# PANXIONG-CN/TEC-MoLLM

Hardware: AMD Instinct MI355X
Metric: train samples/sec (higher is better)
Workload: dtype f32; 1 GPU; BASELINE configs[1]: B=8/GPU, L_in=48, L_out=12, N=2911, F=10 (d_emb=12), 3 GPT-2 blocks, full fwd+bwd+AdamW, fp32, GATv2 per_timestep, dropout on (p=0.1); global_batch=8, parallelism=dp1, data_feed=fixed, launch=eager

## Files before the change

__graft_entry__.py:

```python
from __future__ import annotations

import concurrent.futures as cf
import os
import re
import subprocess
import sys

ROOT = os.path.dirname(os.path.abspath(__file__))
PKG = os.path.join(ROOT, "tec-mollm_amd")
CSRC = os.path.join(PKG, "csrc")
OUT_LIB = os.path.join(PKG, "tecmollm", "libtecmollm_hip.so")
OBJ_DIR = os.path.join(CSRC, "build")
SOURCES = ["gemm.hip", "gemm_mk_nk.hip", "gemm_mk_kn.hip", "gemm_km_kn.hip", "gemm_bf16_mk_nk.hip", "gemm_bf16_mk_kn.hip", "gemm_bf16_km_kn.hip", "gemm_bf16_dma.hip", "gemm_bf16_p8.hip", "gemm_bf16_tn.hip", "gemm_bf16_res_mk.hip", "gemm_bf16_res_km.hip", "gemm_x3.hip", "conv_seq.hip", "conv_dw_seq.hip", "norm.hip", "attention.hip", "attention_long.hip", "spatial_fwd.hip", "spatial_fwd2.hip", "spatial_bwd.hip", "spatial_bwd2.hip", "misc.hip", "trainstep.hip", "baselines.hip", "util.cpp"]
HIPCC = os.environ.get("HIPCC", "/opt/rocm/bin/hipcc")
FLAGS = ["--offload-arch=gfx950", "-O3", "-std=c++17", "-fPIC", "-Wno-pass-failed", "-Wno-unused-value"]


def _ensure_path():
    for p in (ROOT, PKG):
        if p not in sys.path:
            sys.path.insert(0, p)


def _stale(target: str, deps) -> bool:
    if not os.path.exists(target):
        return True
    t = os.path.getmtime(target)
    return any(os.path.getmtime(d) > t for d in deps)


def _compile(src: str) -> str:
    obj = os.path.join(OBJ_DIR, os.path.splitext(src)[0] + ".o")
    deps = [os.path.join(CSRC, src), os.path.join(CSRC, "common.h"), os.path.join(CSRC, "spatial_common.h"), os.path.join(CSRC, "spatial2_common.h"), os.path.join(CSRC, "gemm_impl.h"), os.path.join(CSRC, "gemm_bf16_impl.h"), os.path.join(CSRC, "gemm_x3_impl.h"), os.path.join(CSRC, "gemm_bf16_p8_loop.h"), os.path.join(CSRC, "attention_long.h"), os.path.join(ROOT, "include", "tecmollm.h")]
    if src in SPILL_CEILINGS:
        deps.append(os.path.abspath(__file__))
    if _stale(obj, deps):
        extra = ["-Rpass-analysis=kernel-resource-usage"] if src in SPILL_CEILINGS else []
        cmd = [HIPCC, *FLAGS, *extra, "-x", "hip", "-c", os.path.join(CSRC, src), "-o", obj]
        r = subprocess.run(cmd, capture_output=True, text=True)
        if r.returncode != 0:
            raise RuntimeError(f"hipcc failed on {src}:\n{r.stderr[-4000:]}")
        if src in SPILL_CEILINGS:
            try:
                check_spill_ceilings(src, r.stderr, SPILL_CEILINGS[src])
            except RuntimeError:
                os.remove(obj)
                raise
    return obj


SPILL_CEILINGS = {
    "conv_dw_seq.hip": [("conv_dw_seq_kernel", "ScratchSize [bytes/lane]", 0)],
    "attention.hip": [("attention_bwd_kernel_qstreamILi24ELb0ELb0E", "VGPRs Spill", 92),
                      ("attention_bwd_kernel_qstreamILi24ELb1ELb0E", "VGPRs Spill", 18),
                      ("attention_bwd_kernel_qstreamILi24ELb1ELb1E", "VGPRs Spill", 18)],
    "attention_long.hip": [("att_long_fwd_kernelILb0E", "ScratchSize [bytes/lane]", 0),
                           ("att_long_fwd_kernelILb1E", "ScratchSize [bytes/lane]", 0),
                           ("att_long_bwd_kernelILb0ELb0E", "ScratchSize [bytes/lane]", 0),
                           ("att_long_bwd_kernelILb1ELb0E", "ScratchSize [bytes/lane]", 0),
                           ("att_long_bwd_kernelILb1ELb1E", "ScratchSize [bytes/lane]", 0)],
}


def check_spill_ceilings(src: str, remarks: str, rules) -> None:
    name, bad, seen = None, [], {}
    for line in remarks.splitlines():
        if "Function Name:" in line:
            name = line.split("Function Name:")[1].split()[0]
            continue
        for frag, field, ceiling in rules:
            if name and frag in name and f"{field}:" in line:
                value = int(line.split(f"{field}:")[1].split()[0])
                seen[frag] = seen.get(frag, 0) + 1
                if value > ceiling:
                    bad.append(f"{name}: {field} {value} > {ceiling}")
    missing = [frag for frag, _, _ in rules if not seen.get(frag)]
    if bad or missing:
        raise RuntimeError(f"{src}: kernel resource ceilings exceeded {bad}; no remark for {missing}")


_VREG = re.compile(r"\bv(\d+)\b|\bv\[(\d+):(\d+)\]")


def _vregs(text: str) -> set:
    out = set()
# ... 117 lines not shown
```

include/tecmollm.h:

```cpp
#ifndef TECMOLLM_H
#define TECMOLLM_H

#include <stdint.h>

#ifdef __cplusplus
extern "C" {
#endif

#define TECM_OK 0
#define TECM_E_ARG (-1)
#define TECM_E_ALIGN (-2)
#define TECM_E_LAUNCH (-3)
#define TECM_E_LDS (-4)

#define TECM_ABI_VERSION 19
int tecm_abi_version(void);
const char* tecm_last_error(void);

typedef struct TecmWin {
  int32_t enabled;
  int32_t N;
  int32_t Lin, Lout;
  int32_t stride_t;
  int32_t taps;
  int32_t Cw;
  int32_t pad;
} TecmWin;

typedef struct TecmDrop {
  float p;
  int32_t _pad;
  uint64_t seed;
  int64_t ld;
  const uint64_t* seed_dev;
} TecmDrop;

enum { TECM_A_MK = 0, TECM_A_KM = 1 };
enum { TECM_B_NK = 0, TECM_B_KN = 1 };
enum { TECM_ACT_NONE = 0, TECM_ACT_GELU_ERF = 1, TECM_ACT_GELU_TANH = 2 };

#define TECM_IO_A_BF16 1
#define TECM_IO_B_BF16 2
#define TECM_IO_C_BF16 4
#define TECM_IO_PRE_BF16 8
typedef struct TecmGemm {
  int64_t M, N, K;
  const float* A; int64_t lda; int32_t a_layout; int32_t io_bf16; TecmWin a_win; TecmDrop a_drop;
  const float* B; int64_t ldb; int32_t b_layout; int32_t _p1; TecmWin b_win; TecmDrop b_drop;
// ... 128 lines not shown
int tecm_conv_weight_unpack(const float* dpack, float* dw, int32_t Cout, int32_t Cin, int32_t k,
                            void* stream);

typedef struct TecmConvDx {
  const void* dy;
  const void* wpack;
  float* dinp;
  int32_t B, Lc, N, Cout, ld_in, _pad;
} TecmConvDx;
int tecm_conv_dx_pack(const float* w3, const float* w5, const float* w7, void* wpack, int32_t Cout, int32_t Cin,
                      int32_t ld_in, void* stream);
int tecm_conv_dx_bf16(const TecmConvDx* p, void* stream);
typedef struct TecmConvFwd {
  const void* inp;
  const void* wpack;
  const float* bias;
  float* y;
  int32_t B, Lc, N, Cout, ld_in, y_bf16;
  float* stats;
  float eps;
  int32_t _pad;
} TecmConvFwd;
int tecm_conv_fwd_pack(const float* w3, const float* w5, const float* w7, void* wpack, int32_t Cout, int32_t Cin,
                       int32_t ld_in, void* stream);
int tecm_conv_fwd_bf16(const TecmConvFwd* p, void* stream);
int tecm_conv_fwd_pack_f32(const float* w3, const float* w5, const float* w7, float* wpack, int32_t Cout, int32_t Cin,
                           int32_t ld_in, void* stream);
int tecm_conv_fwd_f32(const TecmConvFwd* p, void* stream);
int tecm_conv_dx_pack_f32(const float* w3, const float* w5, const float* w7, float* wpack, int32_t Cout, int32_t Cin,
                          int32_t ld_in, void* stream);
int tecm_conv_dx_f32(const TecmConvDx* p, void* stream);
int tecm_conv_fwd_supported(int32_t Lc, int32_t Cout, int32_t ld_in, int32_t f32);
int tecm_conv_dx_supported(int32_t Lc, int32_t Cout, int32_t ld_in, int32_t f32);
int tecm_conv_fwd_stats_supported(int32_t Lc);

typedef struct TecmConvDw {
  const void* inp;
  const void* dy;
  float* workspace;
  float* dw3;
  float* dw5;
  float* dw7;
  int32_t B, Lc, N, Cout, Cin, ld_in, num_blocks, _pad;
} TecmConvDw;
int tecm_huber_fwd_bwd_strided(const float* pred, const int64_t* pred_strides , const float* target,
                               const int64_t* target_strides , float* dpred, float* loss_out, int32_t B, int32_t H,
                               int32_t N, float delta, float grad_scale, float* workspace , void* stream);

int64_t tecm_conv_dw_workspace(int32_t Cout, int32_t ld_in, int32_t num_blocks);
int tecm_conv_dw_supported(int32_t Lc, int32_t Cout, int32_t ld_in);
int tecm_conv_dw_bf16(const TecmConvDw* p, void* stream);
int tecm_conv_dw_f32(const TecmConvDw* p, void* stream);

int tecm_cast_bf16(const float* src, int64_t ld_src, void* dst, int64_t ld_dst, int64_t rows, int32_t cols, void* stream);

int tecm_weight_bf16(const float* src, int64_t ld_src, void* same_bf16, int64_t ld_same, void* transposed_bf16, int64_t ld_tr,
                     int32_t rows, int32_t cols, void* stream);

int tecm_dropout_apply(const float* src, int64_t ld_src, void* dst, int64_t ld_dst, int32_t dst_bf16, void* dst2_bf16,
                       int64_t ld_dst2, int64_t rows, int32_t cols, const TecmDrop* drop, void* stream);

int tecm_transpose_scale(const float* src, int64_t lds, float* dst, int64_t ldd, int32_t rows,
                         int32_t cols, float scale, void* stream);

int tecm_lora_fold(const float* lora_B, int32_t n_out, int32_t r, float scale, void* w_kn, int64_t ld_kn, int32_t kn_bf16,
                   void* w_nk, int64_t ld_nk, int32_t nk_bf16, int32_t k_off, void* stream);
// ... 63 lines not shown
```

tec-mollm_amd/csrc/conv_seq.hip:

```cpp
#include "common.h"
#include <type_traits>

typedef float f32x16 __attribute__((ext_vector_type(16)));
typedef __bf16 bf16x8 __attribute__((ext_vector_type(8)));
typedef unsigned int u32x4 __attribute__((ext_vector_type(4)));
typedef float f32x4 __attribute__((ext_vector_type(4)));

namespace tecm_convseq {

#ifndef CDX_ABLATE
#define CDX_ABLATE 0
#endif

constexpr int NB = 4;
constexpr int NTH = 256;
constexpr int MAXT = 6;

__host__ __device__ __forceinline__ int seg_nact(int d) {
  const int a = d < 3 ? 3 - d : d - 3;
  return a <= 1 ? 3 : (a == 2 ? 2 : 1);
}

struct Args {
  const void* dy;
  const void* wpack;
  float* dinp;
  int B, Lc, N, Cout, ld_in, NCI, TC, nchunk, nblk, pitch, zero_off;
  int row_bytes, cpr;
};

struct Tile {
  int b, n0, t0, tc, ts_lo, rows;
};
__device__ __forceinline__ Tile decode_tile(const Args& a, int tile) {
  Tile t;
  const int nbk = tile % a.nblk;
  tile /= a.nblk;
  const int chunk = tile % a.nchunk;
  t.b = tile / a.nchunk;
  t.n0 = nbk * NB;
  t.t0 = chunk * a.TC;
  t.tc = min(a.TC, a.Lc - t.t0);
  t.ts_lo = max(0, t.t0 - 3);
  t.rows = (min(a.Lc, t.t0 + t.tc + 3) - t.ts_lo) * NB;
  return t;
}

template <int SB>
__device__ __forceinline__ void stage_load(const Args& a, const Tile& t, int q0, u32x4 (&v)[SB]) {
  const int cpr = a.cpr, total = t.rows * cpr, nth = (int)blockDim.x;
  const char* src = static_cast<const char*>(a.dy);
#pragma unroll
  for (int q = 0; q < SB; ++q) {
    const int idx = min((int)threadIdx.x + (q0 + q) * nth, total - 1);
    const int row = idx / cpr, ch = idx - row * cpr;
    const int ts = t.ts_lo + (row >> 2);
    const int ng = min(t.n0 + (row & 3), a.N - 1);
    v[q] = *reinterpret_cast<const u32x4*>(src + (((int64_t)t.b * a.Lc + ts) * a.N + ng) * a.row_bytes + ch * 16);
  }
}
template <int SB>
// ... 91 lines not shown
        float* orow = a.dinp + (((int64_t)t.b * a.Lc + tt) * a.N + n) * a.ld_in;
#pragma unroll
        for (int gq = 0; gq < 4; ++gq) {
          const int ci = 32 * c + 8 * gq + 4 * h;
          if (ci < a.ld_in)
            *reinterpret_cast<float4*>(orow + ci) = make_float4(v[4 * gq], v[4 * gq + 1], v[4 * gq + 2], v[4 * gq + 3]);
        }
      }
    }
  }
}

template <int NCI>
__global__ __launch_bounds__(NTH, 2) void conv_dx_seq_kernel(const Args a) {
  extern __shared__ __attribute__((aligned(16))) unsigned char lds[];
  const int tid = threadIdx.x, lane = tid & 63;
  const int wave = __builtin_amdgcn_readfirstlane(tid >> 6);
  const Tile t = decode_tile(a, blockIdx.x);
  {
    constexpr int SB = 12;
    const int total = t.rows * a.cpr;
    for (int q0 = 0; q0 * NTH < ((CDX_ABLATE & 1) ? 0 : total); q0 += SB) {
      u32x4 v[SB];
      stage_load<SB>(a, t, q0, v);
      stage_store<SB>(a, t, q0, v, lds);
    }
    if (tid < a.pitch / 16) *reinterpret_cast<uint4*>(lds + a.zero_off + tid * 16) = make_uint4(0u, 0u, 0u, 0u);
  }
  __syncthreads();
  tile_compute<NCI>(a, t, lds, wave, lane, false);
}

constexpr int NTH32 = 512;

template <int NCI>
__global__ __launch_bounds__(NTH32, 2) void conv_dx_seq_f32_kernel(const Args a) {
  extern __shared__ __attribute__((aligned(16))) unsigned char lds[];
  const int tid = threadIdx.x, lane = tid & 63;
  const int wave = __builtin_amdgcn_readfirstlane(tid >> 6);
  const int r = lane & 31, h = lane >> 5;
  const Tile t = decode_tile(a, blockIdx.x);
  {
    constexpr int SB = 10;
    const int total = t.rows * a.cpr;
    for (int q0 = 0; q0 * NTH32 < total; q0 += SB) {
      u32x4 v[SB];
      stage_load<SB>(a, t, q0, v);
      stage_store<SB>(a, t, q0, v, lds);
    }
    if (tid < a.pitch / 16) *reinterpret_cast<uint4*>(lds + a.zero_off + tid * 16) = make_uint4(0u, 0u, 0u, 0u);
  }
  __syncthreads();

  const int spc = a.Cout / 8;
  const int KS = 15 * spc;
  const int s_beg = wave * (KS / 8), s_end = s_beg + KS / 8;
  int d = 0, sd = s_beg;
  while (sd >= seg_nact(d) * spc) {
    sd -= seg_nact(d) * spc;
    ++d;
  }
  const int ntt = t.tc >> 3;
  f32x16 acc[MAXT];
#pragma unroll
  for (int i = 0; i < MAXT; ++i)
#pragma unroll
    for (int e = 0; e < 16; ++e) acc[i][e] = 0.f;
  const int tl0 = r >> 2;
  constexpr int WD = 3;
  const f32x4* wp = reinterpret_cast<const f32x4*>(a.wpack) + (int64_t)s_beg * NCI * 64 + lane;
  f32x4 wf[WD][NCI];
#pragma unroll
  for (int u = 0; u < WD; ++u)
#pragma unroll
    for (int c = 0; c < NCI; ++c) wf[u][c] = wp[(u * NCI + c) * 64];
  for (int s0 = s_beg; s0 < s_end; s0 += WD) {
#pragma unroll
    for (int u = 0; u < WD; ++u) {
      const int delta = d - 3;
      const int colb = ((3 - seg_nact(d)) * a.Cout + sd * 8 + 4 * h) * 4;
      const int rbase = (t.t0 - t.ts_lo + delta) * 4 + r;
#pragma unroll
      for (int i = 0; i < MAXT / NCI; ++i) {
        if (i < ntt) {
          const int ts = t.t0 + 8 * i + tl0 + delta;
          const bool ok = ts >= 0 && ts < a.Lc;
          const int off = ok ? (rbase + 32 * i) * a.pitch + colb : a.zero_off + 16 * h;
          const f32x4 df = *reinterpret_cast<const f32x4*>(lds + off);
#pragma unroll
          for (int j = 0; j < 4; ++j)
#pragma unroll
            for (int c = 0; c < NCI; ++c)
              acc[i * NCI + c] = __builtin_amdgcn_mfma_f32_32x32x2f32(wf[u][c][j], df[j], acc[i * NCI + c], 0, 0, 0);
        }
      }
      if (s0 + u + WD < s_end) {
#pragma unroll
        for (int c = 0; c < NCI; ++c) wf[u][c] = wp[((u + WD) * NCI + c) * 64];
      }
      if (++sd == seg_nact(d) * spc) {
        sd = 0;
        ++d;
      }
    }
    wp += WD * NCI * 64;
  }
  __syncthreads();

  float* part = reinterpret_cast<float*>(lds);
  const int NT = ntt * NCI;
  if (wave >= 4) {
#pragma unroll
    for (int T = 0; T < MAXT; ++T)
      if (T < NT)
#pragma unroll
        for (int e = 0; e < 16; ++e) part[(((wave - 4) * NT + T) * 16 + e) * 64 + lane] = acc[T][e];
  }
  __syncthreads();
  if (wave < 4) {
#pragma unroll
    for (int T = 0; T < MAXT; ++T)
      if (T < NT)
#pragma unroll
        for (int e = 0; e < 16; ++e) acc[T][e] += part[((wave * NT + T) * 16 + e) * 64 + lane];
  }
  __syncthreads();
  if (wave < 4) {
#pragma unroll
    for (int T = 0; T < MAXT; ++T) {
      if (T < NT && (T & 3) != wave) {
        const int slot = (wave - (T & 3) - 1) & 3;
#pragma unroll
        for (int e = 0; e < 16; ++e) part[((T * 3 + slot) * 16 + e) * 64 + lane] = acc[T][e];
      }
    }
  }
  __syncthreads();
  if (wave < 4) {
#pragma unroll
    for (int T = 0; T < MAXT; ++T) {
      if (T < NT && (T & 3) == wave) {
        f32x16 v = acc[T];
#pragma unroll
        for (int slot = 0; slot < 3; ++slot)
#pragma unroll
          for (int e = 0; e < 16; ++e) v[e] += part[((T * 3 + slot) * 16 + e) * 64 + lane];
        const int i = T / NCI, c = T % NCI;
        const int tt = t.t0 + 8 * i + tl0, n = t.n0 + (r & 3);
        if (n < a.N) {
          float* orow = a.dinp + (((int64_t)t.b * a.Lc + tt) * a.N + n) * a.ld_in;
#pragma unroll
          for (int gq = 0; gq < 4; ++gq) {
            const int ci = 32 * c + 8 * gq + 4 * h;
            if (ci < a.ld_in)
              *reinterpret_cast<float4*>(orow + ci) = make_float4(v[4 * gq], v[4 * gq + 1], v[4 * gq + 2], v[4 * gq + 3]);
          }
        }
      }
    }
  }
}

__global__ __launch_bounds__(256) void conv_dx_pack_f32_kernel(const float* __restrict__ w3, const float* __restrict__ w5,
                                                               const float* __restrict__ w7, float* __restrict__ wpack,
                                                               int Cout, int Cin, int NCI) {
  const int total = 15 * Cout * NCI * 32;
  for (int i = blockIdx.x * 256 + threadIdx.x; i < total; i += gridDim.x * 256) {
    const int j = i & 3, lane = (i >> 2) & 63;
    const int sc = i >> 8, c = sc % NCI, s = sc / NCI;
    int k = 8 * s + 4 * (lane >> 5) + j;
    const int ci = 32 * c + (lane & 31);
    int d = 0;
    while (k >= seg_nact(d) * Cout) {
      k -= seg_nact(d) * Cout;
      ++d;
    }
    const int col = (3 - seg_nact(d)) * Cout + k;
    const int jj = col / Cout, co = col - jj * Cout;
    const int kj = 3 + 2 * jj, tau = (kj - 1) / 2 - (d - 3);
    const float* w = jj == 0 ? w3 : (jj == 1 ? w5 : w7);
    float v = 0.f;
    if (ci < Cin && tau >= 0 && tau < kj) v = w[((int64_t)co * Cin + ci) * kj + tau];
    wpack[i] = v;
  }
}

__global__ __launch_bounds__(256) void conv_dx_pack_kernel(const float* __restrict__ w3, const float* __restrict__ w5,
                                                           const float* __restrict__ w7, __bf16* __restrict__ wpack,
                                                           int Cout, int Cin, int NCI) {
  const int KTOT = 15 * Cout;
  const int total = KTOT * NCI * 32;
  for (int i = blockIdx.x * 256 + threadIdx.x; i < total; i += gridDim.x * 256) {
    const int e = i & 7, lane = (i >> 3) & 63;
    const int sc = i >> 9, c = sc % NCI, s = sc / NCI;
    int k = 16 * s + 8 * (lane >> 5) + e;
    const int ci = 32 * c + (lane & 31);
    int d = 0;
    while (k >= seg_nact(d) * Cout) {
      k -= seg_nact(d) * Cout;
      ++d;
    }
    const int col = (3 - seg_nact(d)) * Cout + k;
    const int j = col / Cout, co = col - j * Cout;
    const int kj = 3 + 2 * j, tau = (kj - 1) / 2 - (d - 3);
    const float* w = j == 0 ? w3 : (j == 1 ? w5 : w7);
    float v = 0.f;
    if (ci < Cin && tau >= 0 && tau < kj) v = w[((int64_t)co * Cin + ci) * kj + tau];
    wpack[i] = (__bf16)v;
  }
}

// ... 475 lines not shown

extern "C" int tecm_conv_fwd_bf16(const TecmConvFwd* p, void* stream) { return conv_fwd_launch(p, stream, false, "tecm_conv_fwd_bf16"); }
extern "C" int tecm_conv_fwd_f32(const TecmConvFwd* p, void* stream) { return conv_fwd_launch(p, stream, true, "tecm_conv_fwd_f32"); }

extern "C" int tecm_conv_fwd_pack_f32(const float* w3, const float* w5, const float* w7, float* wpack, int32_t Cout,
                                      int32_t Cin, int32_t ld_in, void* stream) {
  using namespace tecm_convseq;
  TECM_REQUIRE(w3 && w5 && w7 && wpack, TECM_E_ARG, "tecm_conv_fwd_pack_f32: null pointer");
  TECM_REQUIRE(Cout > 0 && Cout % 32 == 0 && Cout <= 128 && Cin > 0 && Cin <= ld_in && ld_in % 8 == 0, TECM_E_ARG,
               "tecm_conv_fwd_pack_f32: Cout a multiple of 32 up to 128, Cin <= ld_in, ld_in a multiple of 8");
  int tot = 0;
  for (int j = 0; j < 3; ++j) tot += ((3 + 2 * j) * ld_in / 8) * (Cout / 32);
  const int total = tot * 256;
  hipLaunchKernelGGL(conv_fwd_pack_f32_kernel, dim3((total + 255) / 256), dim3(256), 0, (hipStream_t)stream, w3, w5, w7, wpack,
                     Cout, Cin, ld_in);
  TECM_CHECK_LAUNCH("tecm_conv_fwd_pack_f32");
  return TECM_OK;
}

extern "C" int tecm_conv_dx_pack(const float* w3, const float* w5, const float* w7, void* wpack, int32_t Cout, int32_t Cin,
                                 int32_t ld_in, void* stream) {
  using namespace tecm_convseq;
  TECM_REQUIRE(w3 && w5 && w7 && wpack, TECM_E_ARG, "tecm_conv_dx_pack: null pointer");
  TECM_REQUIRE(Cout > 0 && Cout % 64 == 0 && Cin > 0 && Cin <= ld_in && ld_in % 4 == 0, TECM_E_ARG,
               "tecm_conv_dx_pack: Cout must be a multiple of 64, Cin <= ld_in, ld_in a multiple of 4");
  const int NCI = (ld_in + 31) / 32;
  const int total = 15 * Cout * NCI * 32;
  hipLaunchKernelGGL(conv_dx_pack_kernel, dim3((total + 255) / 256), dim3(256), 0, (hipStream_t)stream, w3, w5, w7,
                     static_cast<__bf16*>(wpack), Cout, Cin, NCI);
  TECM_CHECK_LAUNCH("tecm_conv_dx_pack");
  return TECM_OK;
}

struct ConvDxPlan { int TC, zero_off, row_bytes, pitch, NCI; size_t lds; };
static ConvDxPlan conv_dx_plan(int Lc, int Cout, int ld_in, bool f32) {
  using namespace tecm_convseq;
  ConvDxPlan q;
  q.NCI = (ld_in + 31) / 32;
  q.row_bytes = 3 * Cout * (f32 ? 4 : 2);
  q.pitch = q.row_bytes + 16;
  int TC = 8 * (MAXT / q.NCI);
  if (TC > Lc) TC = Lc;
  auto img_steps = [&](int tc) { return tc + 6 < Lc ? tc + 6 : Lc; };
  auto zero_of = [&](int tc) {
    const size_t img = (size_t)img_steps(tc) * NB * q.pitch;
    const size_t xch = (size_t)(tc / 8) * q.NCI * (f32 ? 4 : 3) * 16 * 64 * 4;
    return img > xch ? img : xch;
  };
  while (TC > 8 && zero_of(TC) + q.pitch > 160 * 1024) TC -= 8;
  q.TC = TC;
  q.zero_off = (int)zero_of(TC);
  q.lds = zero_of(TC) + q.pitch;
  return q;
}

extern "C" int tecm_conv_dx_supported(int32_t Lc, int32_t Cout, int32_t ld_in, int32_t f32) {
  if (Lc <= 0 || Lc % 8 != 0 || Cout <= 0 || Cout % 64 != 0 || ld_in <= 0 || ld_in % 4 != 0 || ld_in > 64) return 0;
  return conv_dx_plan(Lc, Cout, ld_in, f32 != 0).lds <= 160 * 1024 ? 1 : 0;
}

static int conv_dx_launch(const TecmConvDx* p, void* stream, bool f32, const char* who) {
  using namespace tecm_convseq;
  TECM_REQUIRE(p && p->dy && p->wpack && p->dinp, TECM_E_ARG, "%s: null pointer", who);
  TECM_REQUIRE(p->B > 0 && p->Lc > 0 && p->N > 0, TECM_E_ARG, "%s: bad shape", who);
  TECM_REQUIRE(p->Cout % 64 == 0 && p->Cout > 0 && p->ld_in % 4 == 0 && p->ld_in > 0 && p->ld_in <= 64, TECM_E_ARG,
               "%s: Cout must be a multiple of 64 and ld_in a multiple of 4 up to 64", who);
  TECM_REQUIRE(p->Lc % 8 == 0, TECM_E_ARG, "%s: the sequence length must be a multiple of 8", who);
  TECM_REQUIRE(tecm_aligned(p->dy, 16) && tecm_aligned(p->wpack, 16) && tecm_aligned(p->dinp, 16), TECM_E_ALIGN,
               "%s: 16-byte aligned pointers", who);
  Args a;
  a.dy = p->dy;
  a.wpack = p->wpack;
  a.dinp = p->dinp;
  a.B = p->B; a.Lc = p->Lc; a.N = p->N; a.Cout = p->Cout; a.ld_in = p->ld_in;
  const ConvDxPlan q = conv_dx_plan(p->Lc, p->Cout, p->ld_in, f32);
  a.NCI = q.NCI;
  a.row_bytes = q.row_bytes;
  a.cpr = a.row_bytes / 16;
  a.pitch = q.pitch;
  const size_t lds = q.lds;
  TECM_REQUIRE(lds <= 160 * 1024, TECM_E_LDS, "%s: %d channels need %zu B of LDS per tile", who, 3 * p->Cout, lds);
  const int TC = q.TC;
  a.TC = TC;
  a.zero_off = q.zero_off;
  a.nchunk = (p->Lc + TC - 1) / TC;
  a.nblk = (p->N + NB - 1) / NB;
  const int64_t tiles = (int64_t)p->B * a.nchunk * a.nblk;
  TECM_REQUIRE(tiles < ((int64_t)1 << 31), TECM_E_ARG, "%s: too many tiles", who);
  const void* fn = f32 ? (a.NCI == 1 ? reinterpret_cast<const void*>(&conv_dx_seq_f32_kernel<1>)
                                     : reinterpret_cast<const void*>(&conv_dx_seq_f32_kernel<2>))
                       : (a.NCI == 1 ? reinterpret_cast<const void*>(&conv_dx_seq_kernel<1>)
                                     : reinterpret_cast<const void*>(&conv_dx_seq_kernel<2>));
  TECM_REQUIRE(hipFuncSetAttribute(fn, hipFuncAttributeMaxDynamicSharedMemorySize, 160 * 1024) == hipSuccess, TECM_E_LAUNCH,
               "%s: hipFuncSetAttribute(MaxDynamicSharedMemorySize) failed", who);
  if (f32) {
    if (a.NCI == 1)
      hipLaunchKernelGGL(conv_dx_seq_f32_kernel<1>, dim3((unsigned)tiles), dim3(NTH32), lds, (hipStream_t)stream, a);
    else
      hipLaunchKernelGGL(conv_dx_seq_f32_kernel<2>, dim3((unsigned)tiles), dim3(NTH32), lds, (hipStream_t)stream, a);
  } else if (a.NCI == 1) {
    hipLaunchKernelGGL(conv_dx_seq_kernel<1>, dim3((unsigned)tiles), dim3(NTH), lds, (hipStream_t)stream, a);
  } else {
    hipLaunchKernelGGL(conv_dx_seq_kernel<2>, dim3((unsigned)tiles), dim3(NTH), lds, (hipStream_t)stream, a);
  }
  TECM_CHECK_LAUNCH("tecm_conv_dx");
  return TECM_OK;
}

extern "C" int tecm_conv_dx_bf16(const TecmConvDx* p, void* stream) { return conv_dx_launch(p, stream, false, "tecm_conv_dx_bf16"); }
extern "C" int tecm_conv_dx_f32(const TecmConvDx* p, void* stream) { return conv_dx_launch(p, stream, true, "tecm_conv_dx_f32"); }

extern "C" int tecm_conv_dx_pack_f32(const float* w3, const float* w5, const float* w7, float* wpack, int32_t Cout,
                                     int32_t Cin, int32_t ld_in, void* stream) {
  using namespace tecm_convseq;
  TECM_REQUIRE(w3 && w5 && w7 && wpack, TECM_E_ARG, "tecm_conv_dx_pack_f32: null pointer");
  TECM_REQUIRE(Cout > 0 && Cout % 64 == 0 && Cin > 0 && Cin <= ld_in && ld_in % 4 == 0, TECM_E_ARG,
               "tecm_conv_dx_pack_f32: Cout must be a multiple of 64, Cin <= ld_in, ld_in a multiple of 4");
  const int NCI = (ld_in + 31) / 32;
  const int total = 15 * Cout * NCI * 32;
  hipLaunchKernelGGL(conv_dx_pack_f32_kernel, dim3((total + 255) / 256), dim3(256), 0, (hipStream_t)stream, w3, w5, w7, wpack,
                     Cout, Cin, NCI);
  TECM_CHECK_LAUNCH("tecm_conv_dx_pack_f32");
  return TECM_OK;
}
```

tec-mollm_amd/tecmollm/_lib.py:

```python
from __future__ import annotations

import ctypes as C
import os
from typing import Optional

import torch

_HERE = os.path.dirname(os.path.abspath(__file__))
LIB_PATH = os.environ.get("TECM_LIB", os.path.join(_HERE, "libtecmollm_hip.so"))
ABI_VERSION = 19

c_f32p = C.c_void_p


class TecmWin(C.Structure):
    _fields_ = [("enabled", C.c_int32), ("N", C.c_int32), ("Lin", C.c_int32), ("Lout", C.c_int32),
                ("stride_t", C.c_int32), ("taps", C.c_int32), ("Cw", C.c_int32), ("pad", C.c_int32)]


class TecmDrop(C.Structure):
    _fields_ = [("p", C.c_float), ("_pad", C.c_int32), ("seed", C.c_uint64), ("ld", C.c_int64), ("seed_dev", C.c_void_p)]


class TecmGemm(C.Structure):
    _fields_ = [
        ("M", C.c_int64), ("N", C.c_int64), ("K", C.c_int64),
        ("A", c_f32p), ("lda", C.c_int64), ("a_layout", C.c_int32), ("io_bf16", C.c_int32),
        ("a_win", TecmWin), ("a_drop", TecmDrop),
        ("B", c_f32p), ("ldb", C.c_int64), ("b_layout", C.c_int32), ("_p1", C.c_int32),
        ("b_win", TecmWin), ("b_drop", TecmDrop),
        ("C", c_f32p), ("ldc", C.c_int64), ("c_win", TecmWin),
        ("alpha", C.c_float), ("act", C.c_int32),
        ("bias", c_f32p),
        ("rowbias", c_f32p), ("rb_ld", C.c_int64), ("rb_div", C.c_int32), ("rb_mod", C.c_int32),
        ("preact", c_f32p), ("ldp", C.c_int64),
        ("dact_src", c_f32p), ("ldd", C.c_int64),
        ("out_drop", TecmDrop),
        ("residual", c_f32p), ("ldr", C.c_int64),
        ("accumulate", C.c_int32), ("split_k", C.c_int32),
        ("workspace", c_f32p),
    ]


# ... 145 lines not shown
    "tecm_cast_bf16": (C.c_int, [c_f32p, C.c_int64, C.c_void_p, C.c_int64, C.c_int64, C.c_int32, C.c_void_p]),
    "tecm_attention_bwd": (C.c_int, [c_f32p, c_f32p, c_f32p, C.c_int32, C.c_int32, C.c_int32, C.c_int32, C.c_int32,
                                     C.c_int32, C.POINTER(TecmDrop), C.c_void_p]),
    "tecm_colsum": (C.c_int, [c_f32p, C.c_int64, C.c_int64, C.c_int64, C.c_int32, C.c_int32, c_f32p, C.c_int64,
                              C.c_int32, C.c_float, C.POINTER(TecmDrop), c_f32p, C.c_void_p]),
    "tecm_colsum_twin": (C.c_int, [c_f32p, C.c_int64, C.c_int64, C.c_int64, C.c_int32, C.c_int32, c_f32p, C.c_int64,
                                   C.c_int32, C.c_float, C.POINTER(TecmDrop), c_f32p, C.c_void_p, C.c_int64, C.c_void_p]),
    "tecm_huber_fwd_bwd": (C.c_int, [c_f32p, c_f32p, c_f32p, c_f32p, C.c_int64, C.c_float, C.c_float, c_f32p,
                                     C.c_void_p]),
    "tecm_huber_fwd_bwd_strided": (C.c_int, [c_f32p, C.POINTER(C.c_int64), c_f32p, C.POINTER(C.c_int64), c_f32p, c_f32p,
                                             C.c_int32, C.c_int32, C.c_int32, C.c_float, C.c_float, c_f32p, C.c_void_p]),
    "tecm_lora_fold": (C.c_int, [c_f32p, C.c_int32, C.c_int32, C.c_float, C.c_void_p, C.c_int64, C.c_int32, C.c_void_p,
                                 C.c_int64, C.c_int32, C.c_int32, C.c_void_p]),
    "tecm_pack_vectors": (C.c_int, [C.POINTER(C.c_void_p), C.POINTER(C.c_int32), C.c_int32, c_f32p, C.c_void_p]),
    "tecm_conv_weight_pack": (C.c_int, [c_f32p, c_f32p, c_f32p, C.c_int32, C.c_int32, C.c_int32, C.c_void_p]),
    "tecm_conv_weight_unpack": (C.c_int, [c_f32p, c_f32p, C.c_int32, C.c_int32, C.c_int32, C.c_void_p]),
    "tecm_conv_dx_pack": (C.c_int, [c_f32p, c_f32p, c_f32p, C.c_void_p, C.c_int32, C.c_int32, C.c_int32, C.c_void_p]),
    "tecm_conv_dx_bf16": (C.c_int, [C.POINTER(TecmConvDx), C.c_void_p]),
    "tecm_conv_fwd_pack": (C.c_int, [c_f32p, c_f32p, c_f32p, C.c_void_p, C.c_int32, C.c_int32, C.c_int32, C.c_void_p]),
    "tecm_conv_fwd_bf16": (C.c_int, [C.POINTER(TecmConvFwd), C.c_void_p]),
    "tecm_conv_fwd_pack_f32": (C.c_int, [c_f32p, c_f32p, c_f32p, c_f32p, C.c_int32, C.c_int32, C.c_int32, C.c_void_p]),
    "tecm_conv_fwd_f32": (C.c_int, [C.POINTER(TecmConvFwd), C.c_void_p]),
    "tecm_conv_dw_workspace": (C.c_int64, [C.c_int32, C.c_int32, C.c_int32]),
    "tecm_conv_dw_supported": (C.c_int, [C.c_int32, C.c_int32, C.c_int32]),
    "tecm_conv_dw_bf16": (C.c_int, [C.POINTER(TecmConvDw), C.c_void_p]),
    "tecm_conv_dw_f32": (C.c_int, [C.POINTER(TecmConvDw), C.c_void_p]),
    "tecm_conv_dx_pack_f32": (C.c_int, [c_f32p, c_f32p, c_f32p, c_f32p, C.c_int32, C.c_int32, C.c_int32, C.c_void_p]),
    "tecm_conv_dx_f32": (C.c_int, [C.POINTER(TecmConvDx), C.c_void_p]),
    "tecm_conv_fwd_supported": (C.c_int, [C.c_int32, C.c_int32, C.c_int32, C.c_int32]),
    "tecm_conv_fwd_stats_supported": (C.c_int, [C.c_int32]),
    "tecm_gemm_tn_splits": (C.c_int32, [C.c_int64, C.c_int64, C.c_int64]),
    "tecm_p8_rows": (C.c_int, [C.c_int64, C.c_int64]),
    "tecm_conv_dx_supported": (C.c_int, [C.c_int32, C.c_int32, C.c_int32, C.c_int32]),
    "tecm_transpose_scale": (C.c_int, [c_f32p, C.c_int64, c_f32p, C.c_int64, C.c_int32, C.c_int32, C.c_float,
                                       C.c_void_p]),
    "tecm_weight_bf16": (C.c_int, [c_f32p, C.c_int64, C.c_void_p, C.c_int64, C.c_void_p, C.c_int64, C.c_int32, C.c_int32,
                                   C.c_void_p]),
    "tecm_dropout_apply": (C.c_int, [c_f32p, C.c_int64, c_f32p, C.c_int64, C.c_int32, C.c_void_p, C.c_int64, C.c_int64,
                                     C.c_int32, C.POINTER(TecmDrop), C.c_void_p]),
    "tecm_adamw_clip_step": (C.c_int, [C.POINTER(TecmAdamW), C.c_void_p]),
    "tecm_checksum_tail": (C.c_int, [c_f32p, C.c_int64, c_f32p, C.c_int32, C.c_int32, C.c_void_p, C.c_void_p]),
    "tecm_checksum_verify": (C.c_int, [c_f32p, C.c_int32, C.c_void_p, C.c_int32, C.c_void_p]),
    "tecm_seed_advance": (C.c_int, [C.c_void_p, C.c_uint64, C.c_void_p]),
    "tecm_metrics_accumulate": (C.c_int, [C.POINTER(TecmMetrics), C.c_void_p]),
    "tecm_window_batch": (C.c_int, [C.POINTER(TecmWindowBatch), C.c_void_p]),
    "tecm_window_baseline": (C.c_int, [C.POINTER(TecmWindowBaseline), C.c_void_p]),
    "tecm_slot_mean": (C.c_int, [C.POINTER(TecmSlotMean), C.c_void_p]),
}

_lib: Optional[C.CDLL] = None


class TecmError(RuntimeError):
    pass


def lib() -> C.CDLL:
    global _lib
    if _lib is not None:
        return _lib
    if not os.path.exists(LIB_PATH):
        raise TecmError(
            f"{LIB_PATH} not found: build it first (python -c 'import __graft_entry__ as g; g.build()'). "
            "The TEC-MoLLM MI355X path has no CPU/PyTorch fallback.")
    handle = C.CDLL(LIB_PATH)
    for name, (res, args) in EXPORTS.items():
# ... 29 lines not shown
```

tec-mollm_amd/tecmollm/ops.py:

```python
from __future__ import annotations

import os
import ctypes as C
from typing import Optional, Tuple

import torch

from . import _lib
from ._lib import TecmDrop, TecmGemm, TecmWin, check, lib, ptr, stream_ptr

A_MK, A_KM = 0, 1
B_NK, B_KN = 0, 1
ACT_NONE, ACT_GELU_ERF, ACT_GELU_TANH = 0, 1, 2

_MASK64 = (1 << 64) - 1


def splitmix64(x: int) -> int:
    x = (x + 0x9E3779B97F4A7C15) & _MASK64
    z = x
    z = ((z ^ (z >> 30)) * 0xBF58476D1CE4E5B9) & _MASK64
    z = ((z ^ (z >> 27)) * 0x94D049BB133111EB) & _MASK64
    return z ^ (z >> 31)

# ... 421 lines not shown
    vecs = [v.detach() for v in vecs]
    if any(v.dtype != torch.float32 or not v.is_contiguous() or v.dim() != 1 for v in vecs) or not 1 <= len(vecs) <= 12:
        raise _lib.TecmError("pack_vectors: 1..12 contiguous fp32 vectors")
    total = sum(v.numel() for v in vecs)
    if out is None:
        out = torch.empty(total, device=vecs[0].device, dtype=torch.float32)
    srcs = (C.c_void_p * len(vecs))(*[v.data_ptr() for v in vecs])
    lens = (C.c_int32 * len(vecs))(*[v.numel() for v in vecs])
    check(lib().tecm_pack_vectors(srcs, lens, len(vecs), out.data_ptr(), stream_ptr()), "tecm_pack_vectors")
    return out


def conv_weight_pack(w: torch.Tensor, want_bwd: bool = True) -> Tuple[torch.Tensor, Optional[torch.Tensor]]:
    Cout, Cin, k = w.shape
    fwd = torch.empty(Cout, k * Cin, device=w.device, dtype=torch.float32)
    bwd = torch.empty(k * Cout, Cin, device=w.device, dtype=torch.float32) if want_bwd else None
    check(lib().tecm_conv_weight_pack(w.data_ptr(), fwd.data_ptr(), ptr(bwd), Cout, Cin, k, stream_ptr()),
          "tecm_conv_weight_pack")
    return fwd, bwd


def conv_weight_unpack(dpack: torch.Tensor, Cout: int, Cin: int, k: int) -> torch.Tensor:
    dw = torch.empty(Cout, Cin, k, device=dpack.device, dtype=torch.float32)
    check(lib().tecm_conv_weight_unpack(dpack.data_ptr(), dw.data_ptr(), Cout, Cin, k, stream_ptr()),
          "tecm_conv_weight_unpack")
    return dw


def conv_dx_seq_ok(Lc: int, Cout: int, ld_in: int, f32: bool = False) -> bool:
    return (os.environ.get("TECM_CONV_SEQ", "1")[:1] != "0"
            and lib().tecm_conv_dx_supported(Lc, Cout, ld_in, 1 if f32 else 0) == 1)


def conv_dx(dy: torch.Tensor, w3: torch.Tensor, w5: torch.Tensor, w7: torch.Tensor, dinp: torch.Tensor, B: int,
            Lc: int, N: int, Cout: int, cin: int, ld_in: int) -> None:
    if dinp.dtype != torch.float32 or dy.dtype not in (torch.bfloat16, torch.float32):
        raise _lib.TecmError("conv_dx: dy is bf16 or fp32, dinp fp32")
    f32 = dy.dtype == torch.float32
    nci = (ld_in + 31) // 32
    wpack = torch.empty(15 * Cout * nci * 32, device=dy.device, dtype=dy.dtype)
    pack, run, what = ((lib().tecm_conv_dx_pack_f32, lib().tecm_conv_dx_f32, "tecm_conv_dx_f32") if f32 else
                       (lib().tecm_conv_dx_pack, lib().tecm_conv_dx_bf16, "tecm_conv_dx_bf16"))
    check(pack(w3.data_ptr(), w5.data_ptr(), w7.data_ptr(), wpack.data_ptr(), Cout, cin, ld_in, stream_ptr()), what + "/pack")
    d = _lib.TecmConvDx(dy=dy.data_ptr(), wpack=wpack.data_ptr(), dinp=dinp.data_ptr(), B=B, Lc=Lc, N=N, Cout=Cout,
                        ld_in=ld_in)
    if _timing is None:
        check(run(C.byref(d), stream_ptr()), what)
        return
    e0, e1 = torch.cuda.Event(enable_timing=True), torch.cuda.Event(enable_timing=True)
    e0.record()
    check(run(C.byref(d), stream_ptr()), what)
    e1.record()
    name = ("conv_dx_seq_f32_kernel" if f32 else "conv_dx_seq_kernel") + \
        (f" M={B * Lc * N} N={ld_in} K={15 * Cout}" if _timing_detail else "")
    _timing.append((name, 2.0 * B * Lc * N * ld_in * 15 * Cout, e0, e1))


conv_dx_bf16 = conv_dx


def conv_dw_seq_ok(Lc: int, Cout: int, ld_in: int) -> bool:
    return os.environ.get("TECM_CONV_DW_SEQ", "1")[:1] != "0" and lib().tecm_conv_dw_supported(Lc, Cout, ld_in) == 1


_cu_count = {}

# ... 78 lines not shown
```

Baseline: 123.8 samples/s.

## Restructure fp32 conv_dx kernel into two channel-half passes for higher occupancy

The fp32 conv input-gradient kernel now stages dy into LDS in two halves of the output channels, shrinking the LDS tile to an 80 KB cap. It splits the K reduction across four waves, with the other two waves covering either the second input-channel chunk or half of the time tiles. It also templates the accumulator count and raises launch bounds to 4 blocks per CU, with spill and VGPR ceilings enforced at build time. The weight pack is reordered per half. The aim is more resident blocks and lower register pressure, at the cost of an extra staging pass and barrier per tile.

Result: no change. 124.6 samples/s, median of 6 (+0.6%).

```diff
diff --git a/__graft_entry__.py b/__graft_entry__.py
--- a/__graft_entry__.py
+++ b/__graft_entry__.py
@@ -51,6 +51,9 @@
 
 SPILL_CEILINGS = {
     "conv_dw_seq.hip": [("conv_dw_seq_kernel", "ScratchSize [bytes/lane]", 0)],
+    "conv_seq.hip": [("conv_dx_seq_f32_kernel", "ScratchSize [bytes/lane]", 0),
+                     ("conv_dx_seq_f32_kernel", "VGPRs", 128),
+                     ("conv_dx_seq_f32_kernel", "AGPRs", 0)],
     "attention.hip": [("attention_bwd_kernel_qstreamILi24ELb0ELb0E", "VGPRs Spill", 92),
                       ("attention_bwd_kernel_qstreamILi24ELb1ELb0E", "VGPRs Spill", 18),
                       ("attention_bwd_kernel_qstreamILi24ELb1ELb1E", "VGPRs Spill", 18)],
diff --git a/include/tecmollm.h b/include/tecmollm.h
--- a/include/tecmollm.h
+++ b/include/tecmollm.h
@@ -13,7 +13,7 @@
 #define TECM_E_LAUNCH (-3)
 #define TECM_E_LDS (-4)
 
-#define TECM_ABI_VERSION 19
+#define TECM_ABI_VERSION 20
 int tecm_abi_version(void);
 const char* tecm_last_error(void);
 
@@ -208,6 +208,8 @@
 int tecm_conv_dx_f32(const TecmConvDx* p, void* stream);
 int tecm_conv_fwd_supported(int32_t Lc, int32_t Cout, int32_t ld_in, int32_t f32);
 int tecm_conv_dx_supported(int32_t Lc, int32_t Cout, int32_t ld_in, int32_t f32);
+int tecm_conv_dx_blocks_per_cu(int32_t Lc, int32_t Cout, int32_t ld_in, int32_t f32);
+int tecm_conv_dx_lds_bytes(int32_t Lc, int32_t Cout, int32_t ld_in, int32_t f32);
 int tecm_conv_fwd_stats_supported(int32_t Lc);
 
 typedef struct TecmConvDw {
diff --git a/tec-mollm_amd/csrc/conv_seq.hip b/tec-mollm_amd/csrc/conv_seq.hip
--- a/tec-mollm_amd/csrc/conv_seq.hip
+++ b/tec-mollm_amd/csrc/conv_seq.hip
@@ -27,6 +27,7 @@
   float* dinp;
   int B, Lc, N, Cout, ld_in, NCI, TC, nchunk, nblk, pitch, zero_off;
   int row_bytes, cpr;
+  int Ch;
 };
 
 struct Tile {
@@ -184,130 +185,143 @@
 }
 
 constexpr int NTH32 = 512;
-
-template <int NCI>
-__global__ __launch_bounds__(NTH32, 2) void conv_dx_seq_f32_kernel(const Args a) {
+constexpr int MAXT32 = 3;
+constexpr int WD32 = 3;
+
+template <int SB>
+__device__ __forceinline__ void stage_pass_f32(const Args& a, const Tile& t, int p, unsigned char* lds) {
+  const int cpr = a.cpr, cpb = a.Ch >> 2, total = t.rows * cpr;
+  const char* src = static_cast<const char*>(a.dy) + (int64_t)p * a.Ch * 4;
+  for (int q0 = 0; q0 * NTH32 < ((CDX_ABLATE & 1) ? 0 : total); q0 += SB) {
+    u32x4 v[SB];
+#pragma unroll
+    for (int q = 0; q < SB; ++q) {
+      const int idx = min((int)threadIdx.x + (q0 + q) * NTH32, total - 1);
+      const int row = idx / cpr, ch = idx - row * cpr;
+      const int j = ch / cpb, wi = ch - j * cpb;
+      const int ts = t.ts_lo + (row >> 2);
+      const int ng = min(t.n0 + (row & 3), a.N - 1);
+      v[q] = *reinterpret_cast<const u32x4*>(src + (((int64_t)t.b * a.Lc + ts) * a.N + ng) * a.row_bytes + (j * a.Cout * 4 + wi * 16));
+    }
+#pragma unroll
+    for (int q = 0; q < SB; ++q) {
+      const int idx = (int)threadIdx.x + (q0 + q) * NTH32;
+      const int row = idx / cpr, ch = idx - row * cpr;
+      if (idx < total) *reinterpret_cast<u32x4*>(lds + row * a.pitch + ch * 16) = v[q];
+    }
+  }
+}
+
+template <int NCI, int NI>
+__device__ __forceinline__ void pass_kloop_f32(const Args& a, const Tile& t, const unsigned char* lds, int p, int kr, int c,
+                                               int i0, int ilast, int lane, f32x16 (&acc)[NI]) {
+  const int r = lane & 31, h = lane >> 5, tl0 = r >> 2;
+  const int spc = a.Ch / 8;
+  const int KS = 15 * spc, per = KS / 4;
+  int d = 0, sd = kr * per;
+  while (sd >= seg_nact(d) * spc) {
+    sd -= seg_nact(d) * spc;
+    ++d;
+  }
+  int rowoff[NI], tsb[NI];
+#pragma unroll
+  for (int ii = 0; ii < NI; ++ii) {
+    const int i = min(i0 + ii, ilast);
+    rowoff[ii] = ((t.t0 - t.ts_lo) * 4 + r + 32 * i) * a.pitch + 16 * h;
+    tsb[ii] = t.t0 + 8 * i + tl0;
+  }
+  const int zoff = a.zero_off + 16 * h;
+  auto rd = [&](f32x4 (&df)[NI]) {
+    const int delta = d - 3;
+    const int soff = delta * 4 * a.pitch + ((3 - seg_nact(d)) * a.Ch + sd * 8) * 4;
+#pragma unroll
+    for (int ii = 0; ii < NI; ++ii) {
+      const bool ok = (unsigned)(tsb[ii] + delta) < (unsigned)a.Lc;
+      const int off = ok ? rowoff[ii] + soff : zoff;
+      df[ii] = *reinterpret_cast<const f32x4*>(lds + off);
+    }
+  };
+  const f32x4* wp = reinterpret_cast<const f32x4*>(a.wpack) + (((int64_t)p * KS + kr * per) * NCI + c) * 64 + lane;
+  f32x4 wq[WD32], df[NI];
+#pragma unroll
+  for (int u = 0; u < WD32; ++u) wq[u] = wp[min(u, per - 1) * NCI * 64];
+  rd(df);
+  for (int s = 0; s < ((CDX_ABLATE & 2) ? 0 : per); ++s) {
+    const f32x4 wn = wp[min(s + WD32, per - 1) * NCI * 64];
+    if (s + 1 < per && ++sd == seg_nact(d) * spc) {
+      sd = 0;
+      ++d;
+    }
+    f32x4 dn[NI];
+    rd(dn);
+#pragma unroll
+    for (int j = 0; j < 4; ++j)
+#pragma unroll
+      for (int ii = 0; ii < NI; ++ii) acc[ii] = __builtin_amdgcn_mfma_f32_32x32x2f32(wq[0][j], df[ii][j], acc[ii], 0, 0, 0);
+#pragma unroll
+    for (int u = 0; u + 1 < WD32; ++u) wq[u] = wq[u + 1];
+    wq[WD32 - 1] = wn;
+#pragma unroll
+    for (int ii = 0; ii < NI; ++ii) df[ii] = dn[ii];
+  }
+}
+
+template <int NCI, int NI>
+__global__ __launch_bounds__(NTH32, 4) void conv_dx_seq_f32_kernel(const Args a) {
   extern __shared__ __attribute__((aligned(16))) unsigned char lds[];
   const int tid = threadIdx.x, lane = tid & 63;
   const int wave = __builtin_amdgcn_readfirstlane(tid >> 6);
+  const int kr = wave & 3, hf = wave >> 2;
   const int r = lane & 31, h = lane >> 5;
   const Tile t = decode_tile(a, blockIdx.x);
-  {
-    constexpr int SB = 10;
-    const int total = t.rows * a.cpr;
-    for (int q0 = 0; q0 * NTH32 < total; q0 += SB) {
-      u32x4 v[SB];
-      stage_load<SB>(a, t, q0, v);
-      stage_store<SB>(a, t, q0, v, lds);
-    }
-    if (tid < a.pitch / 16) *reinterpret_cast<uint4*>(lds + a.zero_off + tid * 16) = make_uint4(0u, 0u, 0u, 0u);
+  const int ntt = t.tc >> 3;
+  const int nloc = NCI == 1 ? (ntt + 1) >> 1 : ntt;
+  const int c = NCI == 1 ? 0 : hf;
+  const int i0 = NCI == 1 ? hf * nloc : 0;
+  const int ni = min(nloc, ntt - i0);
+  f32x16 acc[NI];
+#pragma unroll
+  for (int i = 0; i < NI; ++i)
+#pragma unroll
+    for (int e = 0; e < 16; ++e) acc[i][e] = 0.f;
+  if (tid < a.pitch / 16) *reinterpret_cast<uint4*>(lds + a.zero_off + tid * 16) = make_uint4(0u, 0u, 0u, 0u);
+#pragma unroll 1
+  for (int p = 0; p < 2; ++p) {
+    if (p) __syncthreads();
+    stage_pass_f32<5>(a, t, p, lds);
+    __syncthreads();
+    pass_kloop_f32<NCI, NI>(a, t, lds, p, kr, c, i0, ntt - 1, lane, acc);
   }
   __syncthreads();
 
-  const int spc = a.Cout / 8;
-  const int KS = 15 * spc;
-  const int s_beg = wave * (KS / 8), s_end = s_beg + KS / 8;
-  int d = 0, sd = s_beg;
-  while (sd >= seg_nact(d) * spc) {
-    sd -= seg_nact(d) * spc;
-    ++d;
-  }
-  const int ntt = t.tc >> 3;
-  f32x16 acc[MAXT];
-#pragma unroll
-  for (int i = 0; i < MAXT; ++i)
-#pragma unroll
-    for (int e = 0; e < 16; ++e) acc[i][e] = 0.f;
-  const int tl0 = r >> 2;
-  constexpr int WD = 3;
-  const f32x4* wp = reinterpret_cast<const f32x4*>(a.wpack) + (int64_t)s_beg * NCI * 64 + lane;
-  f32x4 wf[WD][NCI];
-#pragma unroll
-  for (int u = 0; u < WD; ++u)
-#pragma unroll
-    for (int c = 0; c < NCI; ++c) wf[u][c] = wp[(u * NCI + c) * 64];
-  for (int s0 = s_beg; s0 < s_end; s0 += WD) {
-#pragma unroll
-    for (int u = 0; u < WD; ++u) {
-      const int delta = d - 3;
-      const int colb = ((3 - seg_nact(d)) * a.Cout + sd * 8 + 4 * h) * 4;
-      const int rbase = (t.t0 - t.ts_lo + delta) * 4 + r;
-#pragma unroll
-      for (int i = 0; i < MAXT / NCI; ++i) {
-        if (i < ntt) {
-          const int ts = t.t0 + 8 * i + tl0 + delta;
-          const bool ok = ts >= 0 && ts < a.Lc;
-          const int off = ok ? (rbase + 32 * i) * a.pitch + colb : a.zero_off + 16 * h;
-          const f32x4 df = *reinterpret_cast<const f32x4*>(lds + off);
-#pragma unroll
-          for (int j = 0; j < 4; ++j)
-#pragma unroll
-            for (int c = 0; c < NCI; ++c)
-              acc[i * NCI + c] = __builtin_amdgcn_mfma_f32_32x32x2f32(wf[u][c][j], df[j], acc[i * NCI + c], 0, 0, 0);
-        }
-      }
-      if (s0 + u + WD < s_end) {
-#pragma unroll
-        for (int c = 0; c < NCI; ++c) wf[u][c] = wp[((u + WD) * NCI + c) * 64];
-      }
-      if (++sd == seg_nact(d) * spc) {
-        sd = 0;
-        ++d;
-      }
-    }
-    wp += WD * NCI * 64;
+  float* part = reinterpret_cast<float*>(lds) + hf * nloc * 3 * 16 * 64;
+#pragma unroll
+  for (int ii = 0; ii < NI; ++ii) {
+    if (ii < ni && kr != ii && !(CDX_ABLATE & 4)) {
+      const int slot = (kr - ii - 1) & 3;
+#pragma unroll
+      for (int e = 0; e < 16; ++e) part[((ii * 3 + slot) * 16 + e) * 64 + lane] = acc[ii][e];
+    }
   }
   __syncthreads();
-
-  float* part = reinterpret_cast<float*>(lds);
-  const int NT = ntt * NCI;
-  if (wave >= 4) {
-#pragma unroll
-    for (int T = 0; T < MAXT; ++T)
-      if (T < NT)
-#pragma unroll
-        for (int e = 0; e < 16; ++e) part[(((wave - 4) * NT + T) * 16 + e) * 64 + lane] = acc[T][e];
-  }
-  __syncthreads();
-  if (wave < 4) {
-#pragma unroll
-    for (int T = 0; T < MAXT; ++T)
-      if (T < NT)
-#pragma unroll
-        for (int e = 0; e < 16; ++e) acc[T][e] += part[((wave * NT + T) * 16 + e) * 64 + lane];
-  }
-  __syncthreads();
-  if (wave < 4) {
-#pragma unroll
-    for (int T = 0; T < MAXT; ++T) {
-      if (T < NT && (T & 3) != wave) {
-        const int slot = (wave - (T & 3) - 1) & 3;
-#pragma unroll
-        for (int e = 0; e < 16; ++e) part[((T * 3 + slot) * 16 + e) * 64 + lane] = acc[T][e];
-      }
-    }
-  }
-  __syncthreads();
-  if (wave < 4) {
-#pragma unroll
-    for (int T = 0; T < MAXT; ++T) {
-      if (T < NT && (T & 3) == wave) {
-        f32x16 v = acc[T];
-#pragma unroll
-        for (int slot = 0; slot < 3; ++slot)
-#pragma unroll
-          for (int e = 0; e < 16; ++e) v[e] += part[((T * 3 + slot) * 16 + e) * 64 + lane];
-        const int i = T / NCI, c = T % NCI;
-        const int tt = t.t0 + 8 * i + tl0, n = t.n0 + (r & 3);
-        if (n < a.N) {
-          float* orow = a.dinp + (((int64_t)t.b * a.Lc + tt) * a.N + n) * a.ld_in;
-#pragma unroll
-          for (int gq = 0; gq < 4; ++gq) {
-            const int ci = 32 * c + 8 * gq + 4 * h;
-            if (ci < a.ld_in)
-              *reinterpret_cast<float4*>(orow + ci) = make_float4(v[4 * gq], v[4 * gq + 1], v[4 * gq + 2], v[4 * gq + 3]);
-          }
-        }
+  if (kr < ni) {
+    const int ii = kr;
+    f32x16 v = acc[0];
+#pragma unroll
+    for (int u = 1; u < NI; ++u)
+      if (ii == u) v = acc[u];
+#pragma unroll
+    for (int slot = 0; slot < ((CDX_ABLATE & 4) ? 0 : 3); ++slot)
+#pragma unroll
+      for (int e = 0; e < 16; ++e) v[e] += part[((ii * 3 + slot) * 16 + e) * 64 + lane];
+    const int tt = t.t0 + 8 * (i0 + ii) + (r >> 2), n = t.n0 + (r & 3);
+    if (n < a.N) {
+      float* orow = a.dinp + (((int64_t)t.b * a.Lc + tt) * a.N + n) * a.ld_in;
+#pragma unroll
+      for (int gq = 0; gq < 4; ++gq) {
+        const int ci = 32 * c + 8 * gq + 4 * h;
+        if (ci < a.ld_in)
+          *reinterpret_cast<float4*>(orow + ci) = make_float4(v[4 * gq], v[4 * gq + 1], v[4 * gq + 2], v[4 * gq + 3]);
       }
     }
   }
@@ -317,18 +331,20 @@
                                                                const float* __restrict__ w7, float* __restrict__ wpack,
                                                                int Cout, int Cin, int NCI) {
   const int total = 15 * Cout * NCI * 32;
+  const int Ch = Cout / 2, KS = 15 * Ch / 8;
   for (int i = blockIdx.x * 256 + threadIdx.x; i < total; i += gridDim.x * 256) {
     const int j = i & 3, lane = (i >> 2) & 63;
-    const int sc = i >> 8, c = sc % NCI, s = sc / NCI;
+    const int sc = i >> 8, c = sc % NCI, sg = sc / NCI;
+    const int p = sg / KS, s = sg - p * KS;
     int k = 8 * s + 4 * (lane >> 5) + j;
     const int ci = 32 * c + (lane & 31);
     int d = 0;
-    while (k >= seg_nact(d) * Cout) {
-      k -= seg_nact(d) * Cout;
+    while (k >= seg_nact(d) * Ch) {
+      k -= seg_nact(d) * Ch;
       ++d;
     }
-    const int col = (3 - seg_nact(d)) * Cout + k;
-    const int jj = col / Cout, co = col - jj * Cout;
+    const int col = (3 - seg_nact(d)) * Ch + k;
+    const int jj = col / Ch, co = p * Ch + col - jj * Ch;
     const int kj = 3 + 2 * jj, tau = (kj - 1) / 2 - (d - 3);
     const float* w = jj == 0 ? w3 : (jj == 1 ? w5 : w7);
     float v = 0.f;
@@ -870,7 +886,7 @@
   return TECM_OK;
 }
 
-struct ConvDxPlan { int TC, zero_off, row_bytes, pitch, NCI; size_t lds; };
+struct ConvDxPlan { int TC, zero_off, row_bytes, pitch, NCI, NI; size_t lds; };
 static ConvDxPlan conv_dx_plan(int Lc, int Cout, int ld_in, bool f32) {
   using namespace tecm_convseq;
   ConvDxPlan q;
@@ -892,9 +908,46 @@
   return q;
 }
 
+constexpr size_t CONV_DX_F32_LDS = 80 * 1024;
+static ConvDxPlan conv_dx_plan_f32(int Lc, int Cout, int ld_in) {
+  using namespace tecm_convseq;
+  ConvDxPlan q;
+  q.NCI = (ld_in + 31) / 32;
+  q.row_bytes = 3 * Cout * 4;
+  q.pitch = 3 * (Cout / 2) * 4 + 16;
+  auto lds_of = [&](int tc, int* zero) {
+    const size_t img = (size_t)(tc + 6 < Lc ? tc + 6 : Lc) * NB * q.pitch;
+    const int ntt = tc / 8, nloc = q.NCI == 1 ? (ntt + 1) / 2 : ntt;
+    const size_t xch = (size_t)2 * nloc * 3 * 16 * 64 * 4;
+    const size_t z = img > xch ? img : xch;
+    if (zero) *zero = (int)z;
+    return z + q.pitch;
+  };
+  int TC = 8 * (2 * MAXT32 / q.NCI);
+  if (TC > Lc) TC = Lc;
+  while (TC > 8 && lds_of(TC, nullptr) > CONV_DX_F32_LDS) TC -= 8;
+  const int nchunk = (Lc + TC - 1) / TC;
+  TC = ((Lc + nchunk - 1) / nchunk + 7) / 8 * 8;
+  q.TC = TC;
+  q.NI = q.NCI == 1 ? (TC / 8 + 1) / 2 : TC / 8;
+  q.lds = lds_of(TC, &q.zero_off);
+  return q;
+}
+
 extern "C" int tecm_conv_dx_supported(int32_t Lc, int32_t Cout, int32_t ld_in, int32_t f32) {
   if (Lc <= 0 || Lc % 8 != 0 || Cout <= 0 || Cout % 64 != 0 || ld_in <= 0 || ld_in % 4 != 0 || ld_in > 64) return 0;
   return conv_dx_plan(Lc, Cout, ld_in, f32 != 0).lds <= 160 * 1024 ? 1 : 0;
+}
+
+extern "C" int tecm_conv_dx_blocks_per_cu(int32_t Lc, int32_t Cout, int32_t ld_in, int32_t f32) {
+  if (!tecm_conv_dx_supported(Lc, Cout, ld_in, f32)) return 0;
+  const size_t lds = f32 ? conv_dx_plan_f32(Lc, Cout, ld_in).lds : conv_dx_plan(Lc, Cout, ld_in, false).lds;
+  return (int)((size_t)160 * 1024 / lds);
+}
+
+extern "C" int tecm_conv_dx_lds_bytes(int32_t Lc, int32_t Cout, int32_t ld_in, int32_t f32) {
+  if (!tecm_conv_dx_supported(Lc, Cout, ld_in, f32)) return 0;
+  return (int)(f32 ? conv_dx_plan_f32(Lc, Cout, ld_in).lds : conv_dx_plan(Lc, Cout, ld_in, false).lds);
 }
 
 static int conv_dx_launch(const TecmConvDx* p, void* stream, bool f32, const char* who) {
@@ -911,13 +964,17 @@
   a.wpack = p->wpack;
   a.dinp = p->dinp;
   a.B = p->B; a.Lc = p->Lc; a.N = p->N; a.Cout = p->Cout; a.ld_in = p->ld_in;
-  const ConvDxPlan q = conv_dx_plan(p->Lc, p->Cout, p->ld_in, f32);
+  TECM_REQUIRE(!f32 || tecm_conv_dx_supported(p->Lc, p->Cout, p->ld_in, 1), TECM_E_LDS,
+               "%s: %d channels at %d steps are not served in fp32 (tecm_conv_dx_supported)", who, 3 * p->Cout, p->Lc);
+  const ConvDxPlan q = f32 ? conv_dx_plan_f32(p->Lc, p->Cout, p->ld_in) : conv_dx_plan(p->Lc, p->Cout, p->ld_in, false);
   a.NCI = q.NCI;
   a.row_bytes = q.row_bytes;
-  a.cpr = a.row_bytes / 16;
+  a.Ch = p->Cout / 2;
+  a.cpr = (f32 ? 3 * a.Ch * 4 : a.row_bytes) / 16;
   a.pitch = q.pitch;
   const size_t lds = q.lds;
-  TECM_REQUIRE(lds <= 160 * 1024, TECM_E_LDS, "%s: %d channels need %zu B of LDS per tile", who, 3 * p->Cout, lds);
+  TECM_REQUIRE(lds <= (f32 ? CONV_DX_F32_LDS : (size_t)160 * 1024), TECM_E_LDS, "%s: %d channels need %zu B of LDS per tile", who,
+               3 * p->Cout, lds);
   const int TC = q.TC;
   a.TC = TC;
   a.zero_off = q.zero_off;
@@ -925,22 +982,31 @@
   a.nblk = (p->N + NB - 1) / NB;
   const int64_t tiles = (int64_t)p->B * a.nchunk * a.nblk;
   TECM_REQUIRE(tiles < ((int64_t)1 << 31), TECM_E_ARG, "%s: too many tiles", who);
-  const void* fn = f32 ? (a.NCI == 1 ? reinterpret_cast<const void*>(&conv_dx_seq_f32_kernel<1>)
-                                     : reinterpret_cast<const void*>(&conv_dx_seq_f32_kernel<2>))
-                       : (a.NCI == 1 ? reinterpret_cast<const void*>(&conv_dx_seq_kernel<1>)
-                                     : reinterpret_cast<const void*>(&conv_dx_seq_kernel<2>));
-  TECM_REQUIRE(hipFuncSetAttribute(fn, hipFuncAttributeMaxDynamicSharedMemorySize, 160 * 1024) == hipSuccess, TECM_E_LAUNCH,
-               "%s: hipFuncSetAttribute(MaxDynamicSharedMemorySize) failed", who);
+  const dim3 grid((unsigned)tiles);
+  hipStream_t st = (hipStream_t)stream;
+  auto launch = [&](auto kernel, int nth, size_t cap) {
+    if (hipFuncSetAttribute(reinterpret_cast<const void*>(kernel), hipFuncAttributeMaxDynamicSharedMemorySize, (int)cap) != hipSuccess)
+      return false;
+    hipLaunchKernelGGL(kernel, grid, dim3(nth), lds, st, a);
+    return true;
+  };
+  bool ok = false;
   if (f32) {
-    if (a.NCI == 1)
-      hipLaunchKernelGGL(conv_dx_seq_f32_kernel<1>, dim3((unsigned)tiles), dim3(NTH32), lds, (hipStream_t)stream, a);
-    else
-      hipLaunchKernelGGL(conv_dx_seq_f32_kernel<2>, dim3((unsigned)tiles), dim3(NTH32), lds, (hipStream_t)stream, a);
+    TECM_REQUIRE(q.NI >= 1 && q.NI <= MAXT32, TECM_E_ARG, "%s: %d accumulator tiles per wave", who, q.NI);
+    switch (a.NCI * 4 + q.NI) {
+      case 5: ok = launch(conv_dx_seq_f32_kernel<1, 1>, NTH32, CONV_DX_F32_LDS); break;
+      case 6: ok = launch(conv_dx_seq_f32_kernel<1, 2>, NTH32, CONV_DX_F32_LDS); break;
+      case 7: ok = launch(conv_dx_seq_f32_kernel<1, 3>, NTH32, CONV_DX_F32_LDS); break;
+      case 9: ok = launch(conv_dx_seq_f32_kernel<2, 1>, NTH32, CONV_DX_F32_LDS); break;
+      case 10: ok = launch(conv_dx_seq_f32_kernel<2, 2>, NTH32, CONV_DX_F32_LDS); break;
+      default: ok = launch(conv_dx_seq_f32_kernel<2, 3>, NTH32, CONV_DX_F32_LDS); break;
+    }
   } else if (a.NCI == 1) {
-    hipLaunchKernelGGL(conv_dx_seq_kernel<1>, dim3((unsigned)tiles), dim3(NTH), lds, (hipStream_t)stream, a);
+    ok = launch(conv_dx_seq_kernel<1>, NTH, (size_t)160 * 1024);
   } else {
-    hipLaunchKernelGGL(conv_dx_seq_kernel<2>, dim3((unsigned)tiles), dim3(NTH), lds, (hipStream_t)stream, a);
-  }
+    ok = launch(conv_dx_seq_kernel<2>, NTH, (size_t)160 * 1024);
+  }
+  TECM_REQUIRE(ok, TECM_E_LAUNCH, "%s: hipFuncSetAttribute(MaxDynamicSharedMemorySize) failed", who);
   TECM_CHECK_LAUNCH("tecm_conv_dx");
   return TECM_OK;
 }
diff --git a/tec-mollm_amd/tecmollm/_lib.py b/tec-mollm_amd/tecmollm/_lib.py
--- a/tec-mollm_amd/tecmollm/_lib.py
+++ b/tec-mollm_amd/tecmollm/_lib.py
@@ -8,7 +8,7 @@
 
 _HERE = os.path.dirname(os.path.abspath(__file__))
 LIB_PATH = os.environ.get("TECM_LIB", os.path.join(_HERE, "libtecmollm_hip.so"))
-ABI_VERSION = 19
+ABI_VERSION = 20
 
 c_f32p = C.c_void_p
 
@@ -220,6 +220,8 @@
     "tecm_gemm_tn_splits": (C.c_int32, [C.c_int64, C.c_int64, C.c_int64]),
     "tecm_p8_rows": (C.c_int, [C.c_int64, C.c_int64]),
     "tecm_conv_dx_supported": (C.c_int, [C.c_int32, C.c_int32, C.c_int32, C.c_int32]),
+    "tecm_conv_dx_blocks_per_cu": (C.c_int, [C.c_int32, C.c_int32, C.c_int32, C.c_int32]),
+    "tecm_conv_dx_lds_bytes": (C.c_int, [C.c_int32, C.c_int32, C.c_int32, C.c_int32]),
     "tecm_transpose_scale": (C.c_int, [c_f32p, C.c_int64, c_f32p, C.c_int64, C.c_int32, C.c_int32, C.c_float,
                                        C.c_void_p]),
     "tecm_weight_bf16": (C.c_int, [c_f32p, C.c_int64, C.c_void_p, C.c_int64, C.c_void_p, C.c_int64, C.c_int32, C.c_int32,
diff --git a/tec-mollm_amd/tecmollm/ops.py b/tec-mollm_amd/tecmollm/ops.py
--- a/tec-mollm_amd/tecmollm/ops.py
+++ b/tec-mollm_amd/tecmollm/ops.py
@@ -477,6 +477,14 @@
             and lib().tecm_conv_dx_supported(Lc, Cout, ld_in, 1 if f32 else 0) == 1)
 
 
+def conv_dx_blocks_per_cu(Lc: int, Cout: int, ld_in: int, f32: bool = False) -> int:
+    return int(lib().tecm_conv_dx_blocks_per_cu(Lc, Cout, ld_in, 1 if f32 else 0))
+
+
+def conv_dx_lds_bytes(Lc: int, Cout: int, ld_in: int, f32: bool = False) -> int:
+    return int(lib().tecm_conv_dx_lds_bytes(Lc, Cout, ld_in, 1 if f32 else 0))
+
+
 def conv_dx(dy: torch.Tensor, w3: torch.Tensor, w5: torch.Tensor, w7: torch.Tensor, dinp: torch.Tensor, B: int,
             Lc: int, N: int, Cout: int, cin: int, ld_in: int) -> None:
     if dinp.dtype != torch.float32 or dy.dtype not in (torch.bfloat16, torch.float32):
```
